# davidhalladay/Frido

Measured on AMD Instinct MI355X. Metric: images/sec @ DDIM-200, COCO layout2img 256x256, higher is better.
Workload: dtype f16x3 (precision keyword bf16x3: hi/lo fp16 operand planes, 3 MFMA passes, fp32 accumulate: fp32-class); 1 GPU; layout2i f8f4 (configs/frido/layout2i/frido_f8f4_coco_seg.yaml), per-GPU batch 16, DDIM-200 eta=1.0 x 2 stages + MS-VQGAN decode to uint8 images; global_batch=16, parallelism=dp1

## Files before the change

frido_amd/builder.py:

```python
import contextlib
import ctypes as C_

import torch

from . import _lib
from .arch import MH_HEAD_DIMS, check_attention_heads
from .engine import (Operand, POperand, F32, Alias, Pool, Prog, pack_matrix, pack_conv_weight, rup)

ACT_NONE, ACT_RELU, ACT_SILU = 0, 1, 2
GN_FUSED_MAX_HW = 256
SK_DEFER = True
GEMM_PAIR = True
ATTN_FLASH_MIN_KEYS = 512


class Builder:
    def __init__(self, device, nsplit, weights=None, ws_tag="", planes="f16"):
        self.device = torch.device(device)
        self.nsplit = nsplit
        self.planes = planes
        self.ws_tag = ws_tag
        self.w = weights or {}
        self.pool = Pool(self.device)
        self.prog = Prog(self.device, nsplit, ws_tag)
        self._wcache = {}
        self._persist = []
        self.stream_bf16 = nsplit == 1

    @contextlib.contextmanager
    def persist_scope(self):
        outer, mine = self._persist, []
        self._persist = mine
        try:
            yield mine
        finally:
            self._persist = outer

    @contextlib.contextmanager
    def gemm_pair(self):
        if GEMM_PAIR:
            with self.prog.gemm_pair():
                yield
        else:
            yield

    def new_prog(self):
        self.prog = Prog(self.device, self.nsplit, self.ws_tag)
        self.prog.keep.append(self)
        return self.prog

    def f32(self, rows, C):
        return F32(self.pool, rows, C, bf16=self.stream_bf16)

    def f32_strict(self, rows, C):
        return F32(self.pool, rows, C, bf16=False)

    def op(self, rows, K, batch=1):
        return POperand(self.pool, rows, K, self.nsplit, batch=batch)

    def persistent_op(self, rows, K, batch=1, zero=True):
        o = Operand(rows, K, self.nsplit, self.device, zero=zero, batch=batch)
        self._persist.append(o)
        return o

    def persistent_f32(self, *shape, zero=False):
        t = (torch.zeros if zero else torch.empty)(*shape, dtype=torch.float32, device=self.device)
# ... 441 lines not shown
        small = Nk <= 128 and Nq % 16 == 0 and d % 32 == 0 and aligned
        flash = (not small and aligned and (Nk >= ATTN_FLASH_MIN_KEYS or Nk > 4096)
                 and _lib.lib().frido_attn_flash_supported(d))
        if small or flash:
            kind = "FRIDO_OP_ATTN_SMALL" if small else "FRIDO_OP_ATTN_FLASH"
            kw = dict(Q=q.ptr + 2 * q_off, q_lo=q.lo, ldq=ldq, K=k.ptr + 2 * k_off, k_lo=k.lo, k_bs=Nk * ldk, ldk=ldk, VT=vT.ptr,
                      vt_lo=vT.lo, vt_bs=d * Np, ldvt=Np, B=B, Nq=Nq, Nk=Nk, d=d, dv=d, nsplit=self.nsplit, alpha=float(d) ** -0.5)
            if stream:
                res = self.f32(B * Nq, d)
                assert residual is None or getattr(residual, "bf16", False) == res.bf16
                if ln is not None and not res.bf16 and self.nsplit == 2 and (
                        (flash and self._flash_ln_ok(d)) or (small and B * (Nq // 16) >= 256)):
                    n = self.op(B * Nq, d)
                    kw.update(ln_op=n.ptr, ln_lo=n.lo, ld_ln=d, ln_w=self.bias(ln[0] + ".weight"), ln_b=self.bias(ln[0] + ".bias"),
                              ln_eps=ln[1])
                    res.ln_copy = n
                if also_op and small and not res.bf16:
                    o = self.op(B * Nq, d)
                    kw.update(out_op=o.ptr, out_lo=o.lo, ldo=d)
                    res.op_copy = o
                if (stream_dead and small and getattr(res, "op_copy", None) is not None
                        and getattr(res, "ln_copy", None) is not None):
                    kw["skip_act_store"] = 1
                    res.stream_skipped = True
                self.prog.emit(kind, out_act=res.ptr, ld_act=d, residual=residual.ptr if residual is not None else None,
                               ldr=residual.C if residual is not None else 0, bias=bias_ptr, act_bf16=int(res.bf16), **kw)
                return res
            o = self.op(B * Nq, d)
            self.prog.emit(kind, out_op=o.ptr, out_lo=o.lo, ldo=d, **kw)
            return o
        if Nk > 4096:
            raise _lib.FridoHipError(f"attention over {Nk} keys with head dim {d}: the flash kernel is instantiated for "
                                     "d in {128, 256, 384, 512, 576} only and the score-matrix path stops at 4096 keys")
        s = self.f32_strict(B * Nq, Nk)
        self.prog.gemm(Nq, Nk, d, (q.ptr + 2 * q_off, q.lo), (k.ptr + 2 * k_off, k.lo), batch=B, lda=ldq, ldb=ldk,
                       a_bs=Nq * ldq, b_bs=Nk * ldk, alpha=float(d) ** -0.5, out_f32=s.ptr, of_bs=Nq * Nk, ldo=Nk)
        p = self.softmax(s, B * Nq, Nk, Nk, Np)
        s.free()
        if stream:
            res = self.f32(B * Nq, d)
            kw = {}
            if residual is not None:
                kw.update(residual=residual.ptr, ldr=residual.C, res_bs=Nq * residual.C, res_bf16=getattr(residual, "bf16", False))
            self.prog.gemm(Nq, d, Np, p, vT, batch=B, lda=Np, ldb=Np, a_bs=Nq * Np, b_bs=d * Np, bias=bias_ptr, out_f32=res.ptr,
                           of_bs=Nq * d, ldo=d, out_bf16=res.bf16, **kw)
            p.free()
            return res
        o = self.op(B * Nq, d)
        self.prog.gemm(Nq, d, Np, p, vT, batch=B, lda=Np, ldb=Np, a_bs=Nq * Np, b_bs=d * Np, out_op=o.ptr,
                       oo_bs=Nq * d, ldoo=d, oo_lo=o.lo)
        p.free()
        return o

    def attention_heads(self, qkv, ldqkv, vT, B, N, heads, d, *, legacy=True, **one_head):
        C = heads * d
        check_attention_heads(heads, d)
        if heads == 1:
            return self.attention(qkv, ldqkv, qkv, ldqkv, vT, B, N, N, d, q_off=0, k_off=C, **one_head)
        if one_head:
            raise TypeError(f"attention_heads: {sorted(one_head)} apply to the one-head path only")
        k_off, hs = (d, 3 * d) if legacy else (C, d)
        return self.attention_mh(qkv, ldqkv, 0, hs, qkv, ldqkv, k_off, hs, vT, B, N, N, heads, d)

    def attention_mh(self, q, ldq, q_off, q_hs, k, ldk, k_off, k_hs, vT, B, Nq, Nk, heads, d):
        if not _lib.lib().frido_attn_mh_supported(d):
            raise _lib.FridoHipError(f"libfrido_hip.so has no multi-head attention kernel for head dimension {d}")
        C, Np = heads * d, rup(Nk, 32)
        o = self.op(B * Nq, C)
        self.prog.emit("FRIDO_OP_ATTN_MH", Q=q.ptr + 2 * q_off, q_lo=q.lo, ldq=ldq, q_hs=q_hs, K=k.ptr + 2 * k_off, k_lo=k.lo,
                       k_bs=Nk * ldk, ldk=ldk, k_hs=k_hs, VT=vT.ptr, vt_lo=vT.lo, vt_bs=C * Np, ldvt=Np, out_op=o.ptr, out_lo=o.lo,
                       ldo=C, B=B, heads=heads, Nq=Nq, Nk=Nk, d=d, nsplit=self.nsplit, alpha=float(d) ** -0.5)
        return o

    @staticmethod
    def _flash_ln_ok(d):
        L = _lib.lib()
        return bool(L.frido_attn_flash_ln_supported(d))

    def v_transposed(self, x, ldx, wop, B, Nk, d, *, bias_ptr=None, out=None, x_off=0):
        Np = rup(Nk, 32)
        vT = out or self.persistent_op(d, Np, batch=B, zero=True)
        self.prog.gemm(d, Nk, wop.K, wop, (x.ptr + 2 * x_off, x.lo), batch=B, lda=wop.K, ldb=ldx, a_bs=0, b_bs=Nk * ldx,
                       out_op=vT.ptr, oo_bs=d * Np, ldoo=Np, oo_lo=vT.lo, row_bias=bias_ptr)
        return vT
```

frido_amd/csrc/attn.hip:

```cpp
#include "common.h"
#include <atomic>

namespace {

__device__ __forceinline__ bf16x8 ldg8(const frido_bf16* p) { return *reinterpret_cast<const bf16x8*>(p); }

template <int NS>
__device__ __forceinline__ f32x4 mma(const bf16x8 (&a)[2], const bf16x8 (&b)[2], f32x4 acc) {
    if (NS == 2) {
        acc = mfma_op<NS>(a[1], b[0], acc);
        acc = mfma_op<NS>(a[0], b[1], acc);
    }
    return mfma_op<NS>(a[0], b[0], acc);
}

__host__ __device__ constexpr int attn_park_slots(int nw, int g, int ntall) { return ((ntall + nw - 1) / nw + g - 1) / g * g; }
constexpr int attn_lanes_g(int nw, int nf) { return (nw == 16 || (nw == 4 && nf == 2)) ? 2 : 4; }

template <int NS, int NW, int NF>
__global__ __launch_bounds__(NW * 64) void attn_small_kernel(const FridoAttnSmall d) {
    constexpr int G = attn_lanes_g(NW, NF);
    constexpr int SP_LD = NF * 16 + 4, SO_LD = G == 2 ? 48 : G * 16 + 4, P_LD = NF * 16 + 8;
    constexpr bool SO_SWZ = G == 2;
    constexpr int SLD = SP_LD > SO_LD ? SP_LD : SO_LD;
// ... 286 lines not shown
                sat |= op_sat8(y);
                *reinterpret_cast<uint4*>(dst + c) = make_uint4(h[0] | (h[1] << 16), h[2] | (h[3] << 16), h[4] | (h[5] << 16), h[6] | (h[7] << 16));
                *reinterpret_cast<uint4*>(dst + d.ln_lo + c) = make_uint4(l[0] | (l[1] << 16), l[2] | (l[3] << 16), l[4] | (l[5] << 16), l[6] | (l[7] << 16));
            }
        }
    }
    status_raise(sat);
}

template <int NS, int NW, int NF>
bool attn_lds_optin() {
    static std::atomic<uint64_t> done{0};
    int dev = 0;
    if (hipGetDevice(&dev) != hipSuccess) return false;
    const uint64_t bit = 1ull << (dev & 63);
    if (!(done.load(std::memory_order_acquire) & bit)) {
        if (hipFuncSetAttribute(reinterpret_cast<const void*>(&attn_small_kernel<NS, NW, NF>), hipFuncAttributeMaxDynamicSharedMemorySize,
                                16 * (1024 + 4) * (int)sizeof(float)) != hipSuccess)
            return false;
        done.fetch_or(bit, std::memory_order_release);
    }
    return true;
}

template <int NS>
int launch_attn(const FridoAttnSmall& d, hipStream_t s) {
    const int blocks = d.B * (d.Nq / 16);
    const bool many = blocks >= 512;
    const int cs = blocks >= 256 ? 1 : (blocks >= 128 ? 2 : 4);
#define ATTN_LAUNCH(NW, NF)                                                                                               \
    do {                                                                                                                  \
        const size_t dyn = d.ln_op ? (size_t)NW * attn_park_slots(NW, attn_lanes_g(NW, NF), d.dv >> 4) * 1024 : 0;        \
        if (dyn && !attn_lds_optin<NS, NW, NF>()) {                                                                       \
            frido_set_error("attn_small: cannot opt in to %zu bytes of dynamic LDS", dyn);                                \
            return FRIDO_EHIP;                                        \
        }                                                                                                                 \
        hipLaunchKernelGGL((attn_small_kernel<NS, NW, NF>), dim3(blocks, cs), dim3(NW * 64), dyn, s, d);                  \
    } while (0)
    if (d.Nk <= 32) {
        if (many) ATTN_LAUNCH(4, 2); else ATTN_LAUNCH(16, 2);
    } else if (d.Nk <= 64) {
        if (many) ATTN_LAUNCH(4, 4); else ATTN_LAUNCH(8, 4);
    } else {
        ATTN_LAUNCH(4, 8);
    }
#undef ATTN_LAUNCH
    return FRIDO_OK;
}

}

extern "C" int frido_attn_small(const FridoAttnSmall* d, frido_stream_t s) {
    FRIDO_REQUIRE(d && d->Q && d->K && d->VT && (d->out_op || d->out_act), "null pointer");
    FRIDO_REQUIRE(!d->out_act || ((d->ld_act & 3) == 0 && (d->ldr & 3) == 0), "stream strides must be multiples of 4");
    FRIDO_REQUIRE(d->B > 0 && d->Nq > 0 && (d->Nq & 15) == 0, "Nq must be a positive multiple of 16");
    FRIDO_REQUIRE(d->Nk > 0 && d->Nk <= 128 && d->ldvt >= d->Nk && d->ldvt <= 128 && (d->ldvt & 31) == 0, "Nk must be in [1, 128], ldvt a multiple of 32");
    FRIDO_REQUIRE(d->d > 0 && (d->d & 31) == 0 && d->dv > 0 && (d->dv & 15) == 0, "d must be a multiple of 32, dv of 16");
    FRIDO_REQUIRE((d->ldq & 7) == 0 && (d->ldk & 7) == 0 && (d->ldo & 7) == 0 && (d->q_lo & 7) == 0 && (d->k_lo & 7) == 0 &&
                      (d->vt_lo & 7) == 0 && (d->out_lo & 7) == 0 && (d->k_bs & 7) == 0 && (d->vt_bs & 7) == 0,
                  "strides and plane offsets must keep 16-byte alignment");
    FRIDO_REQUIRE(d->nsplit == 1 || d->nsplit == 2, "nsplit must be 1 or 2");
    FRIDO_REQUIRE(!d->skip_act_store || (d->out_act && (d->out_op || d->ln_op)), "skip_act_store: stream form with an operand copy and / or the fused LayerNorm as its consumers");
    FRIDO_REQUIRE(!d->ln_op || (d->out_act && !d->act_bf16 && d->nsplit == 2 && d->B * (d->Nq / 16) >= 256 && d->dv <= 1024 && d->ln_w && d->ln_b &&
                                (d->ld_ln & 7) == 0 && (d->ln_lo & 7) == 0),
                  "ln_op: bf16x3 f32-stream output, B * Nq / 16 >= 256 (one workgroup per 16 rows owns them whole), weight and bias given");
    const int rc = d->nsplit == 2 ? launch_attn<2>(*d, (hipStream_t)s) : launch_attn<1>(*d, (hipStream_t)s);
    if (rc != FRIDO_OK) return rc;
    return frido_check_launch("attn_small");
}
```

frido_amd/csrc/flash.hip:

```cpp
#include "common.h"
#include <atomic>

namespace {

typedef const __attribute__((address_space(1))) void* gptr_t;
typedef __attribute__((address_space(3))) void* lptr_t;

__device__ __forceinline__ bf16x8 lds_read128(unsigned addr) {
    bf16x8 v;
    asm volatile("ds_read_b128 %0, %1" : "=v"(v) : "v"(addr));
    return v;
}

template <int N>
__device__ __forceinline__ void wait_vmcnt() {
    asm volatile("s_waitcnt vmcnt(%0)" ::"n"(N) : "memory");
}
template <int N>
__device__ __forceinline__ void wait_lgkm() {
    asm volatile("s_waitcnt lgkmcnt(%0)" ::"n"(N) : "memory");
    __builtin_amdgcn_sched_barrier(0);
}

template <int NS>
// ... 302 lines not shown
            const int64_t oo = grow * d.ld_act + col;
            if (d.act_bf16)
                *reinterpret_cast<uint2*>(reinterpret_cast<frido_bf16*>(d.out_act) + oo) =
                    make_uint2(f32_to_bf16_bits(v.x) | (f32_to_bf16_bits(v.y) << 16), f32_to_bf16_bits(v.z) | (f32_to_bf16_bits(v.w) << 16));
            else
                *reinterpret_cast<float4*>(reinterpret_cast<float*>(d.out_act) + oo) = v;
            if (ln) {
                o[c] = f32x4{v.x, v.y, v.z, v.w};
                lsum += (v.x + v.y) + (v.z + v.w);
            }
        } else {
            const float vv[4] = {v.x, v.y, v.z, v.w};
            store_op4(d.out_op, d.out_lo, NS, grow * d.ldo + col, vv);
            if (NS == 2) sat |= op_sat4(vv);
        }
    }
    if (ln) {
        const float mean = xor_sum(lsum) * (1.0f / D);
        float q = 0.f;
#pragma unroll
        for (int c = 0; c < CT; ++c) {
            const float a0 = o[c][0] - mean, a1 = o[c][1] - mean, a2 = o[c][2] - mean, a3 = o[c][3] - mean;
            q += (a0 * a0 + a1 * a1) + (a2 * a2 + a3 * a3);
        }
        const float rstd = 1.0f / sqrtf(xor_sum(q) * (1.0f / D) + d.ln_eps);
#pragma unroll
        for (int c = 0; c < CT; ++c) {
            const int col = c * 16 + g * 4;
            const float4 w = *reinterpret_cast<const float4*>(d.ln_w + col), bb = *reinterpret_cast<const float4*>(d.ln_b + col);
            const float y[4] = {(o[c][0] - mean) * rstd * w.x + bb.x, (o[c][1] - mean) * rstd * w.y + bb.y,
                                (o[c][2] - mean) * rstd * w.z + bb.z, (o[c][3] - mean) * rstd * w.w + bb.w};
            store_op4(d.ln_op, d.ln_lo, NS, grow * d.ld_ln + col, y);
            if (NS == 2) sat |= op_sat4(y);
        }
        status_raise(false, g == 0 && stat_bad(mean, rstd));
    }
    status_raise(sat);
}

template <int D>
struct FDGeo {
    static constexpr int NS = 2, NW = 8, BKV = 32;
    static constexpr int KS = D / 32, KSH = KS / 2;
    static constexpr int CT = D / 16, CTH = CT / 2;
    static constexpr int KPL = BKV * D * 2, VPL = D * BKV * 2;
    static constexpr int KBUF = NS * KPL, VBUF = NS * VPL, TILE = KBUF + VBUF;
    static constexpr int XCH = NW * 64 * 8 * 4;
    static constexpr bool KDB = 2 * KBUF + VBUF + XCH <= 163840;
    static constexpr int KSTRIDE = KDB ? KBUF : 0;
    static constexpr int V0 = (KDB ? 2 : 1) * KBUF;
    static constexpr int X0 = V0 + VBUF;
    static constexpr int SMEM = X0 + XCH;
    static constexpr int KP = KS * 2, VP = D / 16;
    static_assert(KS % 2 == 0 && CTH % 2 == 0 && SMEM <= 163840, "d-split geometry / LDS budget");
    static_assert(!KDB || KP % NW == 0, "the counted vmcnt wait of the double-buffered form needs every wave to issue the same number of K pieces");
};

template <int D>
__global__ __launch_bounds__(512, 1) void flash_ds_kernel(const FridoAttnSmall d) {
    using G = FDGeo<D>;
    constexpr int NS = 2, NW = 8, KSH = G::KSH, CTH = G::CTH;
    extern __shared__ __attribute__((aligned(16))) unsigned char smem[];
    const int t = threadIdx.x, lane = t & 63;
    const int wave = __builtin_amdgcn_readfirstlane(t >> 6);
    const int pair = wave >> 1, hf = wave & 1;
    const int r = lane & 15, g = lane >> 4;
    constexpr int BQ = 64;

    const int qblocks = (d.Nq + BQ - 1) / BQ;
    const int nb = qblocks * d.B;
    int bid = blockIdx.x;
    {
        const int q8 = nb >> 3, r8 = nb & 7, xcd = bid & 7, loc = bid >> 3;
        bid = (xcd < r8 ? xcd * (q8 + 1) : r8 * (q8 + 1) + (xcd - r8) * q8) + loc;
    }
    const int z = bid / qblocks, qb = bid - z * qblocks;
    const int q0 = qb * BQ + pair * 16;
    int qrow = q0 + r;
    const bool q_ok = qrow < d.Nq;
    qrow = q_ok ? qrow : d.Nq - 1;
    const int64_t grow = (int64_t)z * d.Nq + qrow;

    bf16x8 qf[KSH][NS];
    {
        const frido_bf16* qp = d.Q + grow * d.ldq + hf * (D / 2) + g * 8;
#pragma unroll
        for (int ks = 0; ks < KSH; ++ks) {
            qf[ks][0] = *reinterpret_cast<const bf16x8*>(qp + ks * 32);
            qf[ks][1] = *reinterpret_cast<const bf16x8*>(qp + d.q_lo + ks * 32);
        }
    }

    const int lrow = lane >> 2;
    const int lq = (lane & 3) ^ ((4 - ((lrow >> 2) & 3)) & 3);
    const int key_l = 8 * (lrow >> 2) + 4 * hf + (lrow & 3);
    const frido_bf16* Kb = d.K + (int64_t)z * d.k_bs + lq * 8;
    const frido_bf16* Vb = d.VT + (int64_t)z * d.vt_bs + (int64_t)lrow * d.ldvt + lq * 8;
    const int ntiles = (d.Nk + G::BKV - 1) / G::BKV;
    auto issue_k = [&](int j) {
        int key = j * G::BKV + key_l;
        key = key < d.Nk ? key : d.Nk - 1;
        const frido_bf16* src = Kb + (int64_t)key * d.ldk;
        unsigned char* dst = smem + (j & 1) * G::KSTRIDE;
#pragma unroll
        for (int i = 0; i < (G::KP + NW - 1) / NW; ++i) {
            const int piece = wave + NW * i;
// ... 105 lines not shown
        }
        float tmax = fmaxf(fmaxf(fmaxf(sv[0], sv[1]), fmaxf(sv[2], sv[3])), fmaxf(fmaxf(sv[4], sv[5]), fmaxf(sv[6], sv[7])));
        tmax = xor_max(tmax);
        const float m_new = fmaxf(m_run, tmax);
        const float corr = __expf(m_run - m_new);
        float pv[8], rs = 0.f;
#pragma unroll
        for (int i = 0; i < 8; ++i) {
            pv[i] = __expf(sv[i] - m_new);
            rs += pv[i];
        }
        rs = xor_sum(rs);
        l_run = l_run * corr + rs;
        m_run = m_new;
        bf16x8 pf[NS];
        {
            uint32_t h[8], l[8];
#pragma unroll
            for (int i = 0; i < 8; i += 2) { split_op2(pv[i], pv[i + 1], NS, h[i], l[i]); h[i + 1] = 0u; l[i + 1] = 0u; }
            u32x4 ph = {h[0] | (h[1] << 16), h[2] | (h[3] << 16), h[4] | (h[5] << 16), h[6] | (h[7] << 16)};
            u32x4 pl = {l[0] | (l[1] << 16), l[2] | (l[3] << 16), l[4] | (l[5] << 16), l[6] | (l[7] << 16)};
            pf[0] = __builtin_bit_cast(bf16x8, ph);
            pf[1] = __builtin_bit_cast(bf16x8, pl);
        }
        if (__any(corr != 1.0f)) {
#pragma unroll
            for (int c = 0; c < CTH; ++c) {
                o[c][0] *= corr; o[c][1] *= corr; o[c][2] *= corr; o[c][3] *= corr;
            }
        }
#pragma unroll
        for (int c = 0; c < CTH; c += 2) {
            const int cur = (c >> 1) & 1;
            if (c + 2 < CTH) {
#pragma unroll
                for (int q = 0; q < 2; ++q)
#pragma unroll
                    for (int p = 0; p < NS; ++p) vf[cur ^ 1][q][p] = lds_read128(v_frag + p * G::VPL + (c + 2 + q) * 1024);
                wait_lgkm<2 * NS>();
            } else {
                wait_lgkm<0>();
            }
            o[c] = mfma_op<NS>(vf[cur][0][1], pf[0], o[c]);
            o[c + 1] = mfma_op<NS>(vf[cur][1][1], pf[0], o[c + 1]);
            o[c] = mfma_op<NS>(vf[cur][0][0], pf[1], o[c]);
            o[c + 1] = mfma_op<NS>(vf[cur][1][0], pf[1], o[c + 1]);
            o[c] = mfma_op<NS>(vf[cur][0][0], pf[0], o[c]);
            o[c + 1] = mfma_op<NS>(vf[cur][1][0], pf[0], o[c + 1]);
            __builtin_amdgcn_sched_barrier(0);
        }
    }

    const float inv = 1.0f / l_run;
    const bool ln = d.ln_op != nullptr;
    float lsum = 0.f;
    bool sat = false;
    if (q_ok) status_raise(false, g == 0 && hf == 0 && stat_bad(m_run, inv));
#pragma unroll
    for (int c = 0; c < CTH; ++c) {
        const int col = (hf * CTH + c) * 16 + g * 4;
        float4 v = make_float4(o[c][0] * inv, o[c][1] * inv, o[c][2] * inv, o[c][3] * inv);
        if (d.out_act) {
            if (d.bias) {
                const float4 bb = *reinterpret_cast<const float4*>(d.bias + col);
                v.x += bb.x; v.y += bb.y; v.z += bb.z; v.w += bb.w;
            }
            if (d.residual) {
                const float4 rr = load_act4(d.residual, grow * d.ldr + col, d.act_bf16);
                v.x += rr.x; v.y += rr.y; v.z += rr.z; v.w += rr.w;
            }
            const int64_t oo = grow * d.ld_act + col;
            if (q_ok) {
                if (d.act_bf16)
                    *reinterpret_cast<uint2*>(reinterpret_cast<frido_bf16*>(d.out_act) + oo) =
                        make_uint2(f32_to_bf16_bits(v.x) | (f32_to_bf16_bits(v.y) << 16), f32_to_bf16_bits(v.z) | (f32_to_bf16_bits(v.w) << 16));
                else
                    *reinterpret_cast<float4*>(reinterpret_cast<float*>(d.out_act) + oo) = v;
            }
            if (ln) {
                o[c] = f32x4{v.x, v.y, v.z, v.w};
                lsum += (v.x + v.y) + (v.z + v.w);
            }
        } else if (q_ok) {
            const float vv[4] = {v.x, v.y, v.z, v.w};
            store_op4(d.out_op, d.out_lo, NS, grow * d.ldo + col, vv);
            sat |= op_sat4(vv);
        }
    }
    if (ln) {
        float* xs = reinterpret_cast<float*>(smem + G::X0);
        const float hs = xor_sum(lsum);
        __builtin_amdgcn_s_barrier();
        if (g == 0) xs[wave * 16 + r] = hs;
        __syncthreads();
        const float mean = (xs[(pair * 2) * 16 + r] + xs[(pair * 2 + 1) * 16 + r]) * (1.0f / D);
        float q = 0.f;
#pragma unroll
        for (int c = 0; c < CTH; ++c) {
            const float a0 = o[c][0] - mean, a1 = o[c][1] - mean, a2 = o[c][2] - mean, a3 = o[c][3] - mean;
            q += (a0 * a0 + a1 * a1) + (a2 * a2 + a3 * a3);
        }
        const float hq = xor_sum(q);
        if (g == 0) xs[128 + wave * 16 + r] = hq;
        __syncthreads();
        const float rstd = 1.0f / sqrtf((xs[128 + (pair * 2) * 16 + r] + xs[128 + (pair * 2 + 1) * 16 + r]) * (1.0f / D) + d.ln_eps);
        if (q_ok) {
#pragma unroll
            for (int c = 0; c < CTH; ++c) {
                const int col = (hf * CTH + c) * 16 + g * 4;
                const float4 w = *reinterpret_cast<const float4*>(d.ln_w + col), bb = *reinterpret_cast<const float4*>(d.ln_b + col);
                const float y[4] = {(o[c][0] - mean) * rstd * w.x + bb.x, (o[c][1] - mean) * rstd * w.y + bb.y,
                                    (o[c][2] - mean) * rstd * w.z + bb.z, (o[c][3] - mean) * rstd * w.w + bb.w};
                store_op4(d.ln_op, d.ln_lo, NS, grow * d.ld_ln + col, y);
                sat |= op_sat4(y);
            }
            status_raise(false, g == 0 && hf == 0 && stat_bad(mean, rstd));
        }
    }
    status_raise(sat);
}

template <int D>
int flash_ds_launch(const FridoAttnSmall& d, hipStream_t s) {
    constexpr int smem = FDGeo<D>::SMEM;
    static std::atomic<uint64_t> done{0};
    int dev = 0;
    if (hipGetDevice(&dev) != hipSuccess) return FRIDO_EHIP;
    const uint64_t bit = 1ull << (dev & 63);
    if (!(done.load(std::memory_order_acquire) & bit)) {
        if (hipFuncSetAttribute(reinterpret_cast<const void*>(&flash_ds_kernel<D>), hipFuncAttributeMaxDynamicSharedMemorySize, smem) != hipSuccess) {
            frido_set_error("attn_flash (d-split): cannot set dynamic LDS size %d", smem);
            return FRIDO_EHIP;
        }
        done.fetch_or(bit, std::memory_order_release);
    }
    const int blocks = d.B * ((d.Nq + 63) / 64);
    hipLaunchKernelGGL((flash_ds_kernel<D>), dim3(blocks), dim3(512), smem, s, d);
    return frido_check_launch("attn_flash(d-split)");
}


template <int D, int NS, int NW, int OS>
int flash_launch(const FridoAttnSmall& d, hipStream_t s) {
    constexpr int smem = FGeo<D, NS, NW, OS>::SMEM;
    static std::atomic<uint64_t> done{0};
    int dev = 0;
    if (hipGetDevice(&dev) != hipSuccess) return FRIDO_EHIP;
    const uint64_t bit = 1ull << (dev & 63);
    if (!(done.load(std::memory_order_acquire) & bit)) {
        if (hipFuncSetAttribute(reinterpret_cast<const void*>(&flash_attn_kernel<D, NS, NW, OS>), hipFuncAttributeMaxDynamicSharedMemorySize,
                                smem) != hipSuccess) {
            frido_set_error("attn_flash: cannot set dynamic LDS size %d", smem);
            return FRIDO_EHIP;
        }
        done.fetch_or(bit, std::memory_order_release);
    }
    const int blocks = d.B * ((d.Nq + NW * 16 - 1) / (NW * 16));
    hipLaunchKernelGGL((flash_attn_kernel<D, NS, NW, OS>), dim3(blocks, OS), dim3(NW * 64), smem, s, d);
    return frido_check_launch("attn_flash");
}

template <int D>
int flash_dispatch(const FridoAttnSmall& d, hipStream_t s) {
    if (d.nsplit == 2) {
        if constexpr (D >= 256 && D <= 512)
            return flash_ds_launch<D>(d, s);
        else
            return flash_launch<D, 2, 4, (D >= 512 ? 2 : 1)>(d, s);
    }
    if constexpr (D <= 384) {
        if ((int64_t)d.B * ((d.Nq + 127) / 128) >= 200) return flash_launch<D, 1, 8, 1>(d, s);
    }
    return flash_launch<D, 1, 4, 1>(d, s);
}

}

extern "C" int frido_attn_flash_supported(int32_t dd) { return dd == 128 || dd == 256 || dd == 384 || dd == 512 || dd == 576; }
extern "C" int frido_attn_flash_ln_supported(int32_t dd) { return dd == 256 || dd == 384 || dd == 512; }

extern "C" int frido_attn_flash(const FridoAttnSmall* d, frido_stream_t s) {
    FRIDO_REQUIRE(d && d->Q && d->K && d->VT && (d->out_op || d->out_act), "null pointer");
    FRIDO_REQUIRE(!d->out_act || ((d->ld_act & 3) == 0 && (d->ldr & 3) == 0), "stream strides must be multiples of 4");
    FRIDO_REQUIRE(d->B > 0 && d->Nq > 0 && d->Nk > 0, "empty problem");
    FRIDO_REQUIRE(d->d == d->dv && frido_attn_flash_supported(d->d), "d = dv must be one of 128, 256, 384, 512, 576");
    FRIDO_REQUIRE(d->ldvt >= ((d->Nk + 31) & ~31) && (d->ldvt & 7) == 0, "V^T rows must be zero-padded to a multiple of 32 keys");
    FRIDO_REQUIRE((d->ldq & 7) == 0 && (d->ldk & 7) == 0 && (d->ldo & 3) == 0 && (d->q_lo & 7) == 0 && (d->k_lo & 7) == 0 &&
                      (d->vt_lo & 7) == 0 && (d->out_lo & 3) == 0 && (d->k_bs & 7) == 0 && (d->vt_bs & 7) == 0,
                  "strides and plane offsets must keep 16-byte alignment");
    FRIDO_REQUIRE(d->nsplit == 1 || d->nsplit == 2, "nsplit must be 1 or 2");
    FRIDO_REQUIRE(!d->skip_act_store, "skip_act_store is served by frido_attn_small only");
    FRIDO_REQUIRE(!d->ln_op || (d->out_act && !d->act_bf16 && d->nsplit == 2 && frido_attn_flash_ln_supported(d->d) && d->ln_w && d->ln_b && (d->ld_ln & 3) == 0 &&
                                (d->ln_lo & 3) == 0),
                  "ln_op: bf16x3 f32-stream output with a head width whose workgroup owns whole rows (frido_attn_flash_ln_supported), weight and bias given");
    hipStream_t st = (hipStream_t)s;
    switch (d->d) {
        case 128: return flash_dispatch<128>(*d, st);
        case 256: return flash_dispatch<256>(*d, st);
        case 384: return flash_dispatch<384>(*d, st);
        case 512: return flash_dispatch<512>(*d, st);
        default: return flash_dispatch<576>(*d, st);
    }
}
```

frido_amd/unet_plan.py:

```python
import numpy as np
import torch

from .arch import unet_arch
from .builder import Builder, ACT_NONE, ACT_RELU, ACT_SILU
from .engine import pack_matrix, rup

import os
X3_SPADE_BF16 = os.environ.get("FRIDO_X3_SPADE_BF16", "0") != "0"
X3_CROSSKV_HI = os.environ.get("FRIDO_X3_CROSSKV_HI", "0") != "0"


class _Shape:

    def __init__(self, C):
        self.C, self.bf16 = C, False


class UNetStagePlan:
    def __init__(self, b: Builder, cfg, *, B, H, W, nctx, stage, x_state, temb_rows, per_sample_t, step_ptr=None,
                 xrep=1, step_bx_ptr=None):
        self.b, self.cfg = b, cfg
        a = self.a = unet_arch(cfg)
        self.B, self.H, self.W, self.nctx, self.stage, self.xrep = B, H, W, nctx, stage, xrep
        self.Bx = B * xrep
# ... 191 lines not shown
        if t1 and t2:
            hmid = b.gn_conv(t1, x1, x2, self.Bx, h, w, n1, 1e-5, pre + ".in_layers.2", gamma=g1, beta=be1, rowvec=rv)
            if has_skip:
                out = b.gn_conv(t2, hmid, None, self.Bx, h, w, n2, 1e-5, pre + ".out_layers.3", gamma=g2, beta=be2,
                                skip=(x1, x2, pre + ".skip_connection"))
            else:
                assert x2 is None
                out = b.gn_conv(t2, hmid, None, self.Bx, h, w, n2, 1e-5, pre + ".out_layers.3", gamma=g2, beta=be2, residual=x1)
            hmid.free()
            return out
        a1, raw = self._norm(x1, x2, HW, pre + ".in_layers.0", 1e-5, ACT_SILU, want_raw=has_skip)
        hmid = b.conv(a1, self.Bx, h, w, pre + ".in_layers.2", rowvec=rv)
        a1.free()
        a2, _ = self._norm(hmid, None, HW, pre + ".out_layers.0", 1e-5, ACT_SILU, x1_dead=True)
        hmid.free()
        if has_skip and raw.K % 64 == 0 and a2.K % 64 == 0:
            out = b.conv_plus_skip(a2, raw, self.Bx, h, w, pre + ".out_layers.3", pre + ".skip_connection")
            raw.free()
        elif has_skip:
            res = b.linear(raw, pre + ".skip_connection")
            raw.free()
            out = b.conv(a2, self.Bx, h, w, pre + ".out_layers.3", residual=res, out=("f32", res))
        else:
            assert x2 is None
            out = b.conv(a2, self.Bx, h, w, pre + ".out_layers.3", residual=x1)
        a2.free()
        return out

    def _spatial_transformer(self, blk, x, h, w):
        b, HW, C, Bx = self.b, h * w, blk.cin, self.Bx
        pre = blk.prefix
        a0, _ = self._norm(x, None, HW, pre + ".norm", 1e-6, ACT_NONE)
        hcur = b.linear(a0, pre + ".proj_in")
        a0.free()
        depth = self.a.transformer_depth
        for dpt in range(depth):
            hcur = self._transformer_block(pre, dpt, hcur, x if dpt == depth - 1 else None, HW, C)
        return hcur

    def _transformer_block(self, pre, dpt, hcur, x, HW, C):
        b, Bx = self.b, self.Bx
        last = x is not None
        t = f"{pre}.transformer_blocks.{dpt}"
        n1 = b.layernorm(hcur, t + ".norm1")
        wq, _ = b.folded_qk_weight(t + ".attn1.to_q", t + ".attn1.to_k", "q")
        Np = rup(HW, 32)
        if (C, HW) not in self._vt_self:
            self._vt_self[(C, HW)] = b.persistent_op(C, Np, batch=Bx, zero=True)
        vT = self._vt_self[(C, HW)]
        wvo, bvo = b.folded_vo_weight(t + ".attn1.to_v", t + ".attn1.to_out.0")
        with b.gemm_pair():
            b.v_transposed(n1, C, wvo, Bx, HW, C, out=vT)
            qp = b.linear(n1, None, wop=wq, bias=False, out="op")
        h2 = b.attention(qp, C, n1, C, vT, Bx, HW, HW, C, bias_ptr=bvo, residual=hcur, stream=True, ln=(t + ".norm2", 1e-5))
        qp.free()
        n1.free()
        hcur.free()
        n2 = getattr(h2, "ln_copy", None)
        if n2 is None:
            n2 = b.layernorm(h2, t + ".norm2")
        kc, vTc, bvo2 = self.kv[(pre, dpt)]
        chain = last and C % 64 == 0
        h3 = b.attention(n2, C, kc, C, vTc, Bx, HW, self.nctx, C, bias_ptr=bvo2, residual=h2, stream=True, also_op=chain,
                         ln=(t + ".norm3", 1e-5), stream_dead=chain)
        n2.free()
        h2.free()
        n3 = getattr(h3, "ln_copy", None)
        if n3 is None:
            n3 = b.layernorm(h3, t + ".norm3")
        gg = b.linear_geglu(n3, t + ".ff.net.0.proj")
        n3.free()
        if not last:
            out = b.linear(gg, t + ".ff.net.2", residual=h3)
            gg.free()
            h3.free()
            return out
        h3op = h3 if b.stream_bf16 else getattr(h3, "op_copy", None)
        if chain and h3op is not None:
            out = b.chained_linear(gg, h3op, t + ".ff.net.2", pre + ".proj_out", x)
            gg.free()
            if h3op is not h3:
                h3op.free()
            h3.free()
            return out
        assert not getattr(h3, "stream_skipped", False)
        h4 = b.linear(gg, t + ".ff.net.2", residual=h3, out="op")
        gg.free()
        h3.free()
        out = b.linear(h4, pre + ".proj_out", residual=x)
        h4.free()
        return out

    def _attention_block(self, blk, x, h, w):
        b, HW, C, Bx = self.b, h * w, blk.cin, self.Bx
        pre, heads = blk.prefix, blk.heads
        d = C // heads
        a0, _ = self._norm(x, None, HW, pre + ".norm", 1e-5, ACT_NONE)
        if (C, HW) not in self._vt_self:
            self._vt_self[(C, HW)] = b.persistent_op(C, rup(HW, 32), batch=Bx, zero=True)
        vT = self._vt_self[(C, HW)]
        hh, jj = torch.arange(heads)[:, None], torch.arange(d)[None, :]
        vrows = ((2 * C + hh * d + jj) if (blk.new_order or heads == 1) else (3 * d * hh + 2 * d + jj)).flatten()
        key = ("attn_v", pre, heads == 1)
        if key not in b._wcache:
            wqkv, bqkv = b.h64(pre + ".qkv.weight"), b.h64(pre + ".qkv.bias")
            wv, bv = wqkv[vrows], bqkv[vrows]
            if heads == 1:
                wo = b.h64(pre + ".proj_out.weight")
                wv, bv = wo @ wv, wo @ bv + b.h64(pre + ".proj_out.bias")
            b._wcache[key] = (pack_matrix(b.to_dev(wv), b.nsplit), b.to_dev(bv))
        wv_op, bv_dev = b._wcache[key]
        with b.gemm_pair():
            b.v_transposed(a0, C, wv_op, Bx, HW, C, bias_ptr=None if heads == 1 else bv_dev.data_ptr(), out=vT)
            if heads == 1:
                qk = b.linear(a0, None, wop=b.lin_weight(pre + ".qkv.weight", rows=(0, 2 * C)), bias_ptr=b.bias(pre + ".qkv.bias"), out="op")
            else:
                qkv = b.linear(a0, pre + ".qkv", out="op")
        if heads == 1:
            out = b.attention(qk, 2 * C, qk, 2 * C, vT, Bx, HW, HW, C, q_off=0, k_off=C, bias_ptr=bv_dev.data_ptr(), residual=x, stream=True)
# ... 122 lines not shown
```

include/frido_hip.h:

```cpp
#ifndef FRIDO_HIP_H
#define FRIDO_HIP_H

#include <stdint.h>

#ifdef __cplusplus
extern "C" {
#endif

typedef void* frido_stream_t;
typedef uint16_t frido_bf16;

#define FRIDO_ABI_VERSION 8
#define FRIDO_SPLITK_HEADER_BYTES 65536

#define FRIDO_OK 0
#define FRIDO_EINVAL (-1)
#define FRIDO_EHIP (-2)
#define FRIDO_EUNSUPPORTED (-3)

enum { FRIDO_ACT_NONE = 0, FRIDO_ACT_RELU = 1, FRIDO_ACT_SILU = 2, FRIDO_ACT_GELU = 3 ,
       FRIDO_ACT_QUICKGELU = 4  };

typedef struct FridoGemm {
    int32_t M, N, K, batch;
// ... 35 lines not shown
    const float* w_f32;
} FridoGemm;

typedef struct FridoGnStats {
    const float* x1; int32_t C1; const float* x2; int32_t C2;
    int32_t B, HW, groups, nsplit_px;
    double* partials;
    int32_t x_bf16;
    const float* p1; const float* p2;
} FridoGnStats;

typedef struct FridoGnApply {
    const float* x1; int32_t C1; const float* x2; int32_t C2;
    int32_t B, HW, groups, nsplit_px;
    const double* partials; float eps;
    const float* weight; const float* bias;
    const float* gamma; const float* beta;
    int32_t act; int32_t nsplit;
    frido_bf16* out_op; int64_t out_lo;
    frido_bf16* raw_op; int64_t raw_lo;
    float* out_f32;
    int32_t x_bf16;
    int32_t gb_bf16;
    const float* sk_ws; int32_t sk_n; float sk_alpha;
    const float* sk_bias; const float* sk_rowvec; const int32_t* sk_rowvec_step; int32_t sk_rows_per_vec, sk_ldv;
    const float* sk_residual; int32_t sk_ldr;
    float* sk_out;
} FridoGnApply;

typedef struct FridoLayerNorm {
    const float* x; int32_t rows, C; float eps;
    const float* weight; const float* bias;
    int32_t nsplit; frido_bf16* out_op; int64_t out_lo;
    int32_t x_bf16;
    float* out_f32;
} FridoLayerNorm;

typedef struct FridoSoftmax {
    const float* x; int32_t rows, N, ld, Npad;
    int32_t nsplit; frido_bf16* out_op; int64_t out_lo;
    int32_t causal_nq;
} FridoSoftmax;

typedef struct FridoAttnSmall {
    const frido_bf16* Q; int64_t q_lo; int32_t ldq;
    const frido_bf16* K; int64_t k_lo; int64_t k_bs; int32_t ldk;
    const frido_bf16* VT; int64_t vt_lo; int64_t vt_bs; int32_t ldvt;
    frido_bf16* out_op; int64_t out_lo; int32_t ldo;
    int32_t B, Nq, Nk, d, dv, nsplit; float alpha;
    void* out_act; const void* residual; const float* bias; int32_t ld_act, ldr, act_bf16;
    frido_bf16* ln_op; int64_t ln_lo; int32_t ld_ln;
    const float* ln_w; const float* ln_b; float ln_eps;
    int32_t skip_act_store;
} FridoAttnSmall;

typedef struct FridoAttnMh {
    const frido_bf16* Q; int64_t q_lo; int32_t ldq, q_hs;
    const frido_bf16* K; int64_t k_lo; int64_t k_bs; int32_t ldk, k_hs;
    const frido_bf16* VT; int64_t vt_lo; int64_t vt_bs; int32_t ldvt;
    frido_bf16* out_op; int64_t out_lo; int32_t ldo;
    int32_t B, heads, Nq, Nk, d, nsplit; float alpha;
} FridoAttnMh;

typedef struct FridoGeglu {
    const float* x; int32_t rows, H;
    int32_t nsplit; frido_bf16* out_op; int64_t out_lo;
} FridoGeglu;

typedef struct FridoPack {
    const float* src; int32_t B, HW, Csrc, c0, Cuse, Cpad, nchw;
    float scale;
    int32_t nsplit; frido_bf16* out_op; int64_t out_lo;
} FridoPack;

typedef struct FridoRelayout {
    const float* src; float* dst;
    int32_t B, HW, Csrc, c0, Cuse, Cdst, d0, to_nchw;
} FridoRelayout;

typedef struct FridoVq {
    const float* x; int32_t npix, Cx, c0, e;
    float inv_scale;
    const float* codebook; int32_t n_codes;
    float* zq; int32_t Cq, q0;
    int64_t* idx;
    const int64_t* force_idx;
} FridoVq;

typedef struct FridoSamplerStep {
    float* x; int32_t B, HW, Cx, start, nch;
    const float* eps_cond; const float* eps_uncond; float cfg_scale;
    float* eps_out;
    const float* hist1; const float* hist2; const float* hist3;
    const float* coef; const int32_t* step; int32_t coef_row_offset;
    const float* noise; int64_t noise_stride; int32_t noise_C, noise_c0;
    uint64_t seed; int64_t sample0; int32_t rng_stream;
    const int64_t* rng_dev;
    float temperature;
    float* x_out;
    float* pred_x0;
    int32_t write_x;
    const float* cfg_dev;
    float* hist_ring; int64_t hist_stride; int32_t hist_mode;
} FridoSamplerStep;
#define FRIDO_STEP_ANCESTRAL 16

// ... 185 lines not shown
```

Baseline: 3.453 images/s.

## Fuse cross-attention and second LayerNorm into the flash self-attention epilogue

Adds a cross-attention tail to the row-owning d-split flash kernel, enabled for head widths 256 and 384 with at most 32 context keys. After self-attention, bias, residual and norm2, the kernel keeps the normalized rows in registers and computes the small cross-attention (Q·K2, softmax, P·V2) with MFMA. It then adds bias2 and the residual, applies norm3, and writes the results directly. This removes a separate cross-attention launch and the global round-trips of h2 and n2 per transformer block. In exchange it raises register and LDS pressure in the flash epilogue and adds many new ABI fields and validation checks.

Measured after the change: 3.496 images/s, median of 6. +1.2%, better.

```diff
diff --git a/frido_amd/builder.py b/frido_amd/builder.py
--- a/frido_amd/builder.py
+++ b/frido_amd/builder.py
@@ -12,6 +12,8 @@
 SK_DEFER = True
 GEMM_PAIR = True
 ATTN_FLASH_MIN_KEYS = 512
+ATTN_CHAIN = True
+ATTN_CHAIN_HEAD_DIMS = (256, 384)
 
 
 class Builder:
@@ -559,6 +561,34 @@
         p.free()
         return o
 
+    def attention_chain_ok(self, ldq, ldk, Nk, d, Nk2, ldk2):
+        return bool(ATTN_CHAIN and self.nsplit == 2 and not self.stream_bf16 and d in ATTN_CHAIN_HEAD_DIMS and self._flash_ln_ok(d)
+                    and Nk >= ATTN_FLASH_MIN_KEYS and ldq % 8 == 0 and ldk % 8 == 0 and ldk2 % 8 == 0 and 1 <= Nk2 <= 32)
+
+    def attention_chain(self, q, ldq, k, ldk, vT, B, Nq, Nk, d, *, bias_ptr, residual, ln, k2, ldk2, vT2, Nk2, bias2_ptr, ln2,
+                        also_op=False, stream_dead=False):
+        assert self.attention_chain_ok(ldq, ldk, Nk, d, Nk2, ldk2) and residual is not None and not getattr(residual, "bf16", False)
+        Np = rup(Nk, 32)
+        res = self.f32(B * Nq, d)
+        n3 = self.op(B * Nq, d)
+        res.ln_copy = n3
+        kw = dict(Q=q.ptr, q_lo=q.lo, ldq=ldq, K=k.ptr, k_lo=k.lo, k_bs=Nk * ldk, ldk=ldk, VT=vT.ptr, vt_lo=vT.lo, vt_bs=d * Np, ldvt=Np,
+                  B=B, Nq=Nq, Nk=Nk, d=d, dv=d, nsplit=self.nsplit, alpha=float(d) ** -0.5, residual=residual.ptr, ldr=residual.C,
+                  bias=bias_ptr, ln_w=self.bias(ln[0] + ".weight"), ln_b=self.bias(ln[0] + ".bias"), ln_eps=ln[1],
+                  K2=k2.ptr, k2_lo=k2.lo, k2_bs=Nk2 * ldk2, ldk2=ldk2, VT2=vT2.ptr, vt2_lo=vT2.lo, vt2_bs=d * 32, ldvt2=32, Nk2=Nk2,
+                  alpha2=float(d) ** -0.5, bias2=bias2_ptr, ln2_w=self.bias(ln2[0] + ".weight"), ln2_b=self.bias(ln2[0] + ".bias"),
+                  ln2_eps=ln2[1], ln2_op=n3.ptr, ln2_lo=n3.lo, ld_ln2=d)
+        if also_op:
+            o = self.op(B * Nq, d)
+            kw.update(out2_op=o.ptr, out2_lo=o.lo, ldo2=d)
+            res.op_copy = o
+        if stream_dead and also_op:
+            res.stream_skipped = True
+        else:
+            kw.update(out2_act=res.ptr, ld_act2=d)
+        self.prog.emit("FRIDO_OP_ATTN_FLASH", **kw)
+        return res
+
     def attention_heads(self, qkv, ldqkv, vT, B, N, heads, d, *, legacy=True, **one_head):
         C = heads * d
         check_attention_heads(heads, d)
diff --git a/frido_amd/csrc/attn.hip b/frido_amd/csrc/attn.hip
--- a/frido_amd/csrc/attn.hip
+++ b/frido_amd/csrc/attn.hip
@@ -362,6 +362,7 @@
 
 extern "C" int frido_attn_small(const FridoAttnSmall* d, frido_stream_t s) {
     FRIDO_REQUIRE(d && d->Q && d->K && d->VT && (d->out_op || d->out_act), "null pointer");
+    FRIDO_REQUIRE(!d->K2 && !d->VT2 && !d->Nk2 && !d->ln2_op && !d->out2_op && !d->out2_act, "cross tail (K2 ...) is served by frido_attn_flash only");
     FRIDO_REQUIRE(!d->out_act || ((d->ld_act & 3) == 0 && (d->ldr & 3) == 0), "stream strides must be multiples of 4");
     FRIDO_REQUIRE(d->B > 0 && d->Nq > 0 && (d->Nq & 15) == 0, "Nq must be a positive multiple of 16");
     FRIDO_REQUIRE(d->Nk > 0 && d->Nk <= 128 && d->ldvt >= d->Nk && d->ldvt <= 128 && (d->ldvt & 31) == 0, "Nk must be in [1, 128], ldvt a multiple of 32");
diff --git a/frido_amd/csrc/flash.hip b/frido_amd/csrc/flash.hip
--- a/frido_amd/csrc/flash.hip
+++ b/frido_amd/csrc/flash.hip
@@ -378,6 +378,8 @@
     static constexpr int X0 = V0 + VBUF;
     static constexpr int SMEM = X0 + XCH;
     static constexpr int KP = KS * 2, VP = D / 16;
+    static constexpr bool TAIL = D <= 384;
+    static_assert(!TAIL || KBUF >= XCH + 1024, "the tail's exchange words live in the first K buffer");
     static_assert(KS % 2 == 0 && CTH % 2 == 0 && SMEM <= 163840, "d-split geometry / LDS budget");
     static_assert(!KDB || KP % NW == 0, "the counted vmcnt wait of the double-buffered form needs every wave to issue the same number of K pieces");
 };
@@ -589,7 +591,10 @@
     }
 
     const float inv = 1.0f / l_run;
-    const bool ln = d.ln_op != nullptr;
+    const frido_bf16* k2_ptr = d.K2;
+    asm volatile("" : "+s"(k2_ptr));
+    const bool tail = G::TAIL && k2_ptr != nullptr;
+    const bool ln = d.ln_op != nullptr || tail;
     float lsum = 0.f;
     bool sat = false;
     if (q_ok) status_raise(false, g == 0 && hf == 0 && stat_bad(m_run, inv));
@@ -597,7 +602,7 @@
     for (int c = 0; c < CTH; ++c) {
         const int col = (hf * CTH + c) * 16 + g * 4;
         float4 v = make_float4(o[c][0] * inv, o[c][1] * inv, o[c][2] * inv, o[c][3] * inv);
-        if (d.out_act) {
+        if (d.out_act || tail) {
             if (d.bias) {
                 const float4 bb = *reinterpret_cast<const float4*>(d.bias + col);
                 v.x += bb.x; v.y += bb.y; v.z += bb.z; v.w += bb.w;
@@ -607,7 +612,7 @@
                 v.x += rr.x; v.y += rr.y; v.z += rr.z; v.w += rr.w;
             }
             const int64_t oo = grow * d.ld_act + col;
-            if (q_ok) {
+            if (q_ok && d.out_act) {
                 if (d.act_bf16)
                     *reinterpret_cast<uint2*>(reinterpret_cast<frido_bf16*>(d.out_act) + oo) =
                         make_uint2(f32_to_bf16_bits(v.x) | (f32_to_bf16_bits(v.y) << 16), f32_to_bf16_bits(v.z) | (f32_to_bf16_bits(v.w) << 16));
@@ -622,6 +627,32 @@
             const float vv[4] = {v.x, v.y, v.z, v.w};
             store_op4(d.out_op, d.out_lo, NS, grow * d.ldo + col, vv);
             sat |= op_sat4(vv);
+        }
+    }
+    bf16x8 k2f[G::TAIL ? CTH / 2 : 1][2][NS];
+    constexpr int K2E = CTH / 2 <= 4 ? CTH / 2 : 2;
+    const frido_bf16* k2p[2] = {nullptr, nullptr};
+    auto load_k2 = [&](int ks) {
+#pragma unroll
+        for (int f = 0; f < 2; ++f)
+#pragma unroll
+            for (int p = 0; p < NS; ++p) {
+                const frido_bf16* src = k2p[f] + (p ? d.k2_lo : 0) + ks * 32;
+                const uint2 a0 = *reinterpret_cast<const uint2*>(src), a1 = *reinterpret_cast<const uint2*>(src + 16);
+                k2f[ks][f][p] = __builtin_bit_cast(bf16x8, u32x4{a0.x, a0.y, a1.x, a1.y});
+            }
+    };
+    if constexpr (G::TAIL) {
+        if (tail) {
+            const frido_bf16* k2b = k2_ptr + (int64_t)z * d.k2_bs + hf * (D / 2) + g * 4;
+            int key0 = 8 * (r >> 2) + (r & 3), key1 = key0 + 4;
+            key0 = key0 < d.Nk2 ? key0 : d.Nk2 - 1;
+            key1 = key1 < d.Nk2 ? key1 : d.Nk2 - 1;
+            const frido_bf16* kp[2] = {k2b + (int64_t)key0 * d.ldk2, k2b + (int64_t)key1 * d.ldk2};
+            k2p[0] = kp[0];
+            k2p[1] = kp[1];
+#pragma unroll
+            for (int ks = 0; ks < K2E; ++ks) load_k2(ks);
         }
     }
     if (ln) {
@@ -641,17 +672,154 @@
         if (g == 0) xs[128 + wave * 16 + r] = hq;
         __syncthreads();
         const float rstd = 1.0f / sqrtf((xs[128 + (pair * 2) * 16 + r] + xs[128 + (pair * 2 + 1) * 16 + r]) * (1.0f / D) + d.ln_eps);
-        if (q_ok) {
+        if (!tail) {
+            if (q_ok) {
+#pragma unroll
+                for (int c = 0; c < CTH; ++c) {
+                    const int col = (hf * CTH + c) * 16 + g * 4;
+                    const float4 w = *reinterpret_cast<const float4*>(d.ln_w + col), bb = *reinterpret_cast<const float4*>(d.ln_b + col);
+                    const float y[4] = {(o[c][0] - mean) * rstd * w.x + bb.x, (o[c][1] - mean) * rstd * w.y + bb.y,
+                                        (o[c][2] - mean) * rstd * w.z + bb.z, (o[c][3] - mean) * rstd * w.w + bb.w};
+                    store_op4(d.ln_op, d.ln_lo, NS, grow * d.ld_ln + col, y);
+                    sat |= op_sat4(y);
+                }
+                status_raise(false, g == 0 && hf == 0 && stat_bad(mean, rstd));
+            }
+        } else if constexpr (G::TAIL) {
+            if (q_ok) status_raise(false, g == 0 && hf == 0 && stat_bad(mean, rstd));
+            uint32_t nh[CTH][2], nl[CTH][2];
 #pragma unroll
             for (int c = 0; c < CTH; ++c) {
                 const int col = (hf * CTH + c) * 16 + g * 4;
                 const float4 w = *reinterpret_cast<const float4*>(d.ln_w + col), bb = *reinterpret_cast<const float4*>(d.ln_b + col);
                 const float y[4] = {(o[c][0] - mean) * rstd * w.x + bb.x, (o[c][1] - mean) * rstd * w.y + bb.y,
                                     (o[c][2] - mean) * rstd * w.z + bb.z, (o[c][3] - mean) * rstd * w.w + bb.w};
-                store_op4(d.ln_op, d.ln_lo, NS, grow * d.ld_ln + col, y);
+                split_op2(y[0], y[1], NS, nh[c][0], nl[c][0]);
+                split_op2(y[2], y[3], NS, nh[c][1], nl[c][1]);
                 sat |= op_sat4(y);
-            }
-            status_raise(false, g == 0 && hf == 0 && stat_bad(mean, rstd));
+                if (q_ok && d.ln_op) {
+                    const int64_t no = grow * d.ld_ln + col;
+                    *reinterpret_cast<uint2*>(d.ln_op + no) = make_uint2(nh[c][0], nh[c][1]);
+                    *reinterpret_cast<uint2*>(d.ln_op + d.ln_lo + no) = make_uint2(nl[c][0], nl[c][1]);
+                }
+            }
+            f32x4 t0 = f32x4{0.f, 0.f, 0.f, 0.f}, t1 = t0;
+            {
+                __builtin_amdgcn_sched_barrier(0);
+#pragma unroll
+                for (int ks = K2E; ks < CTH / 2; ++ks) load_k2(ks);
+#pragma unroll
+                for (int c = 0; c < CTH; c += 2) {
+                    const bf16x8(&ka)[2][NS] = k2f[c / 2];
+                    const bf16x8 bh = __builtin_bit_cast(bf16x8, u32x4{nh[c][0], nh[c][1], nh[c + 1][0], nh[c + 1][1]});
+                    const bf16x8 bl = __builtin_bit_cast(bf16x8, u32x4{nl[c][0], nl[c][1], nl[c + 1][0], nl[c + 1][1]});
+                    t0 = mfma_op<NS>(ka[0][0], bl, t0);
+                    t1 = mfma_op<NS>(ka[1][0], bl, t1);
+                    t0 = mfma_op<NS>(ka[0][1], bh, t0);
+                    t1 = mfma_op<NS>(ka[1][1], bh, t1);
+                    t0 = mfma_op<NS>(ka[0][0], bh, t0);
+                    t1 = mfma_op<NS>(ka[1][0], bh, t1);
+                }
+            }
+            f32x4* xt = reinterpret_cast<f32x4*>(smem);
+            float* xs2 = reinterpret_cast<float*>(smem + G::XCH);
+            __builtin_amdgcn_sched_barrier(0);
+            bf16x8 v2f[CTH][NS];
+            {
+                const frido_bf16* v2b = d.VT2 + (int64_t)z * d.vt2_bs + (int64_t)(hf * (D / 2) + r) * d.ldvt2 + g * 8;
+#pragma unroll
+                for (int c = 0; c < CTH; ++c) {
+                    const frido_bf16* src = v2b + (int64_t)c * 16 * d.ldvt2;
+                    v2f[c][0] = *reinterpret_cast<const bf16x8*>(src);
+                    v2f[c][1] = *reinterpret_cast<const bf16x8*>(src + d.vt2_lo);
+                }
+            }
+            xt[(wave * 64 + lane) * 2] = t0;
+            xt[(wave * 64 + lane) * 2 + 1] = t1;
+            __syncthreads();
+            const f32x4 u0 = xt[((wave ^ 1) * 64 + lane) * 2], u1 = xt[((wave ^ 1) * 64 + lane) * 2 + 1];
+            const float a2 = d.alpha2;
+            float sv[8] = {(t0[0] + u0[0]) * a2, (t0[1] + u0[1]) * a2, (t0[2] + u0[2]) * a2, (t0[3] + u0[3]) * a2,
+                           (t1[0] + u1[0]) * a2, (t1[1] + u1[1]) * a2, (t1[2] + u1[2]) * a2, (t1[3] + u1[3]) * a2};
+#pragma unroll
+            for (int i = 0; i < 8; ++i)
+                if (8 * g + i >= d.Nk2) sv[i] = -1.0e30f;
+            float mx = fmaxf(fmaxf(fmaxf(sv[0], sv[1]), fmaxf(sv[2], sv[3])), fmaxf(fmaxf(sv[4], sv[5]), fmaxf(sv[6], sv[7])));
+            mx = xor_max(mx);
+            float pv[8], rs = 0.f;
+#pragma unroll
+            for (int i = 0; i < 8; ++i) {
+                pv[i] = __expf(sv[i] - mx);
+                rs += pv[i];
+            }
+            const float inv2 = 1.0f / xor_sum(rs);
+            if (q_ok) status_raise(false, g == 0 && hf == 0 && stat_bad(mx, inv2));
+            bf16x8 pf[NS];
+            {
+                uint32_t h[4], l[4];
+#pragma unroll
+                for (int i = 0; i < 4; ++i) split_op2(pv[2 * i] * inv2, pv[2 * i + 1] * inv2, NS, h[i], l[i]);
+                pf[0] = __builtin_bit_cast(bf16x8, u32x4{h[0], h[1], h[2], h[3]});
+                pf[1] = __builtin_bit_cast(bf16x8, u32x4{l[0], l[1], l[2], l[3]});
+            }
+            float lsum2 = 0.f;
+#pragma unroll
+            for (int c = 0; c < CTH; ++c) {
+                f32x4 acc = f32x4{0.f, 0.f, 0.f, 0.f};
+                acc = mfma_op<NS>(v2f[c][0], pf[1], acc);
+                acc = mfma_op<NS>(v2f[c][1], pf[0], acc);
+                acc = mfma_op<NS>(v2f[c][0], pf[0], acc);
+                if (d.bias2) {
+                    const float4 bb = *reinterpret_cast<const float4*>(d.bias2 + (hf * CTH + c) * 16 + g * 4);
+                    acc[0] += bb.x; acc[1] += bb.y; acc[2] += bb.z; acc[3] += bb.w;
+                }
+                o[c] = f32x4{acc[0] + o[c][0], acc[1] + o[c][1], acc[2] + o[c][2], acc[3] + o[c][3]};
+                lsum2 += (o[c][0] + o[c][1]) + (o[c][2] + o[c][3]);
+            }
+            __builtin_amdgcn_sched_barrier(0);
+            float4 w2f[CTH];
+            if (d.ln2_op) {
+#pragma unroll
+                for (int c = 0; c < CTH; ++c) w2f[c] = *reinterpret_cast<const float4*>(d.ln2_w + (hf * CTH + c) * 16 + g * 4);
+            }
+            const float hs2 = xor_sum(lsum2);
+            if (g == 0) xs2[wave * 16 + r] = hs2;
+            if (q_ok && (d.out2_op || d.out2_act)) {
+#pragma unroll
+                for (int c = 0; c < CTH; ++c) {
+                    const int col = (hf * CTH + c) * 16 + g * 4;
+                    const float vv[4] = {o[c][0], o[c][1], o[c][2], o[c][3]};
+                    if (d.out2_act) *reinterpret_cast<float4*>(d.out2_act + grow * d.ld_act2 + col) = make_float4(vv[0], vv[1], vv[2], vv[3]);
+                    if (d.out2_op) {
+                        store_op4(d.out2_op, d.out2_lo, NS, grow * d.ldo2 + col, vv);
+                        sat |= op_sat4(vv);
+                    }
+                }
+            }
+            __syncthreads();
+            const float mean2 = (xs2[(pair * 2) * 16 + r] + xs2[(pair * 2 + 1) * 16 + r]) * (1.0f / D);
+            float q2 = 0.f;
+#pragma unroll
+            for (int c = 0; c < CTH; ++c) {
+                const float a0 = o[c][0] - mean2, a1 = o[c][1] - mean2, a2c = o[c][2] - mean2, a3 = o[c][3] - mean2;
+                q2 += (a0 * a0 + a1 * a1) + (a2c * a2c + a3 * a3);
+            }
+            const float hq2 = xor_sum(q2);
+            if (g == 0) xs2[128 + wave * 16 + r] = hq2;
+            __syncthreads();
+            const float rstd2 = 1.0f / sqrtf((xs2[128 + (pair * 2) * 16 + r] + xs2[128 + (pair * 2 + 1) * 16 + r]) * (1.0f / D) + d.ln2_eps);
+            if (q_ok && d.ln2_op) {
+#pragma unroll
+                for (int c = 0; c < CTH; ++c) {
+                    const int col = (hf * CTH + c) * 16 + g * 4;
+                    const float4 w = w2f[c], bb = *reinterpret_cast<const float4*>(d.ln2_b + col);
+                    const float y[4] = {(o[c][0] - mean2) * rstd2 * w.x + bb.x, (o[c][1] - mean2) * rstd2 * w.y + bb.y,
+                                        (o[c][2] - mean2) * rstd2 * w.z + bb.z, (o[c][3] - mean2) * rstd2 * w.w + bb.w};
+                    store_op4(d.ln2_op, d.ln2_lo, NS, grow * d.ld_ln2 + col, y);
+                    sat |= op_sat4(y);
+                }
+                status_raise(false, g == 0 && hf == 0 && stat_bad(mean2, rstd2));
+            }
         }
     }
     status_raise(sat);
@@ -717,8 +885,22 @@
 extern "C" int frido_attn_flash_ln_supported(int32_t dd) { return dd == 256 || dd == 384 || dd == 512; }
 
 extern "C" int frido_attn_flash(const FridoAttnSmall* d, frido_stream_t s) {
-    FRIDO_REQUIRE(d && d->Q && d->K && d->VT && (d->out_op || d->out_act), "null pointer");
-    FRIDO_REQUIRE(!d->out_act || ((d->ld_act & 3) == 0 && (d->ldr & 3) == 0), "stream strides must be multiples of 4");
+    FRIDO_REQUIRE(d && d->Q && d->K && d->VT && (d->out_op || d->out_act || d->K2), "null pointer");
+    const bool tail = d->K2 != nullptr;
+    FRIDO_REQUIRE(tail || (!d->VT2 && !d->Nk2 && !d->bias2 && !d->ln2_w && !d->ln2_b && !d->ln2_op && !d->out2_op && !d->out2_act),
+                  "cross tail: fields set without K2 (an absent tail is all zero)");
+    FRIDO_REQUIRE(!tail || (d->nsplit == 2 && (d->d == 256 || d->d == 384)),
+                  "cross tail: two-plane mode and a head width of the row-owning d-split kernel that carries it (256, 384)");
+    FRIDO_REQUIRE(!tail || (!d->out_op && !d->act_bf16 && d->residual), "cross tail: the f32 stream form with a residual (out_op unset; out_act may be null = not stored)");
+    FRIDO_REQUIRE(!tail || (d->ln_w && d->ln_b && (!d->ln2_op || (d->ln2_w && d->ln2_b))), "cross tail: LayerNorm weight and bias given (ln_w, ln_b; ln2_w, ln2_b with ln2_op)");
+    FRIDO_REQUIRE(!tail || (d->VT2 && d->Nk2 >= 1 && d->Nk2 <= 32 && d->ldvt2 >= 32), "cross tail: 1 <= Nk2 <= 32, V2^T rows zero-padded to 32 keys");
+    FRIDO_REQUIRE(!tail || ((d->ldk2 & 7) == 0 && (d->k2_lo & 7) == 0 && (d->k2_bs & 7) == 0 && (d->ldvt2 & 7) == 0 && (d->vt2_lo & 7) == 0 && (d->vt2_bs & 7) == 0 &&
+                            (d->ldo2 & 3) == 0 && (d->out2_lo & 3) == 0 && (d->ld_ln2 & 3) == 0 && (d->ln2_lo & 3) == 0 && (d->ld_act2 & 3) == 0 &&
+                            (d->ld_ln & 3) == 0 && (d->ln_lo & 3) == 0 && aligned16(d->K2) && aligned16(d->VT2) && aligned16(d->bias2) && aligned16(d->ln2_w) &&
+                            aligned16(d->ln2_b) && aligned16(d->out2_act)),
+                  "cross tail: strides, plane offsets and pointers must keep 16-byte alignment");
+    FRIDO_REQUIRE(!tail || d->out2_op || d->out2_act || d->ln2_op, "cross tail: at least one of out2_op, out2_act, ln2_op");
+    FRIDO_REQUIRE(!(d->out_act || tail) || ((d->ld_act & 3) == 0 && (d->ldr & 3) == 0), "stream strides must be multiples of 4");
     FRIDO_REQUIRE(d->B > 0 && d->Nq > 0 && d->Nk > 0, "empty problem");
     FRIDO_REQUIRE(d->d == d->dv && frido_attn_flash_supported(d->d), "d = dv must be one of 128, 256, 384, 512, 576");
     FRIDO_REQUIRE(d->ldvt >= ((d->Nk + 31) & ~31) && (d->ldvt & 7) == 0, "V^T rows must be zero-padded to a multiple of 32 keys");
@@ -727,7 +909,7 @@
                   "strides and plane offsets must keep 16-byte alignment");
     FRIDO_REQUIRE(d->nsplit == 1 || d->nsplit == 2, "nsplit must be 1 or 2");
     FRIDO_REQUIRE(!d->skip_act_store, "skip_act_store is served by frido_attn_small only");
-    FRIDO_REQUIRE(!d->ln_op || (d->out_act && !d->act_bf16 && d->nsplit == 2 && frido_attn_flash_ln_supported(d->d) && d->ln_w && d->ln_b && (d->ld_ln & 3) == 0 &&
+    FRIDO_REQUIRE(!d->ln_op || ((d->out_act || tail) && !d->act_bf16 && d->nsplit == 2 && frido_attn_flash_ln_supported(d->d) && d->ln_w && d->ln_b && (d->ld_ln & 3) == 0 &&
                                 (d->ln_lo & 3) == 0),
                   "ln_op: bf16x3 f32-stream output with a head width whose workgroup owns whole rows (frido_attn_flash_ln_supported), weight and bias given");
     hipStream_t st = (hipStream_t)s;
diff --git a/frido_amd/unet_plan.py b/frido_amd/unet_plan.py
--- a/frido_amd/unet_plan.py
+++ b/frido_amd/unet_plan.py
@@ -267,19 +267,26 @@
         with b.gemm_pair():
             b.v_transposed(n1, C, wvo, Bx, HW, C, out=vT)
             qp = b.linear(n1, None, wop=wq, bias=False, out="op")
-        h2 = b.attention(qp, C, n1, C, vT, Bx, HW, HW, C, bias_ptr=bvo, residual=hcur, stream=True, ln=(t + ".norm2", 1e-5))
-        qp.free()
-        n1.free()
-        hcur.free()
-        n2 = getattr(h2, "ln_copy", None)
-        if n2 is None:
-            n2 = b.layernorm(h2, t + ".norm2")
         kc, vTc, bvo2 = self.kv[(pre, dpt)]
         chain = last and C % 64 == 0
-        h3 = b.attention(n2, C, kc, C, vTc, Bx, HW, self.nctx, C, bias_ptr=bvo2, residual=h2, stream=True, also_op=chain,
-                         ln=(t + ".norm3", 1e-5), stream_dead=chain)
-        n2.free()
-        h2.free()
+        if b.attention_chain_ok(C, C, HW, C, self.nctx, C):
+            h3 = b.attention_chain(qp, C, n1, C, vT, Bx, HW, HW, C, bias_ptr=bvo, residual=hcur, ln=(t + ".norm2", 1e-5), k2=kc, ldk2=C,
+                                   vT2=vTc, Nk2=self.nctx, bias2_ptr=bvo2, ln2=(t + ".norm3", 1e-5), also_op=chain, stream_dead=chain)
+            qp.free()
+            n1.free()
+            hcur.free()
+        else:
+            h2 = b.attention(qp, C, n1, C, vT, Bx, HW, HW, C, bias_ptr=bvo, residual=hcur, stream=True, ln=(t + ".norm2", 1e-5))
+            qp.free()
+            n1.free()
+            hcur.free()
+            n2 = getattr(h2, "ln_copy", None)
+            if n2 is None:
+                n2 = b.layernorm(h2, t + ".norm2")
+            h3 = b.attention(n2, C, kc, C, vTc, Bx, HW, self.nctx, C, bias_ptr=bvo2, residual=h2, stream=True, also_op=chain,
+                             ln=(t + ".norm3", 1e-5), stream_dead=chain)
+            n2.free()
+            h2.free()
         n3 = getattr(h3, "ln_copy", None)
         if n3 is None:
             n3 = b.layernorm(h3, t + ".norm3")
diff --git a/include/frido_hip.h b/include/frido_hip.h
--- a/include/frido_hip.h
+++ b/include/frido_hip.h
@@ -111,6 +111,13 @@
     frido_bf16* ln_op; int64_t ln_lo; int32_t ld_ln;
     const float* ln_w; const float* ln_b; float ln_eps;
     int32_t skip_act_store;
+    const frido_bf16* K2; int64_t k2_lo; int64_t k2_bs; int32_t ldk2;
+    const frido_bf16* VT2; int64_t vt2_lo; int64_t vt2_bs; int32_t ldvt2;
+    int32_t Nk2; float alpha2; const float* bias2;
+    const float* ln2_w; const float* ln2_b; float ln2_eps;
+    frido_bf16* ln2_op; int64_t ln2_lo; int32_t ld_ln2;
+    frido_bf16* out2_op; int64_t out2_lo; int32_t ldo2;
+    float* out2_act; int32_t ld_act2;
 } FridoAttnSmall;
 
 typedef struct FridoAttnMh {
```
